# jyjblrd/Low-Cost-Mocap

Measured on AMD Instinct MI355X. Metric: triangulated 3D markers/sec at 8 cams x 16 markers, higher is better.
Workload: dtype f64

## Files before the change

### low-cost-mocap_amd/csrc/frame_bb.hip

```cpp
#include "mocap_device.hpp"
#include "kernels.hpp"
#include <cstdlib>
#include "frame_common.hpp"

namespace mocap {

constexpr int kBBThreads = 256;
constexpr int kBBWaves = kBBThreads / 64;
constexpr int kBBRecs = kBBThreads + 64;

constexpr int bb_wg_per_cu(int RL) { return RL == 48 ? 5 : 4; }
constexpr int kBBLdsSlack = 1024;
struct BBLayout {
  size_t bxy, bxy_nx, cnt_nx, bt, rbound, seedkey, slot_key, claimw, recs, rpk, scr, scr_bytes, goff, gcnt, outslot, boff, bnb, seedgh, slot_g, cnt,
      misc, bpl, nh, hits, act, root_blob, root_cam, nact, bnl, bv, bcache, bpk, total;
  int ncache;
  __host__ __device__ static size_t al(size_t x, size_t a) { return (x + a - 1) / a * a; }
  __host__ __device__ BBLayout(int C, int M, int R, int CW, int wg_per_cu) {
    size_t o = 0;
    auto take = [&](size_t bytes, size_t a) {
      o = al(o, a);
      const size_t at = o;
      o += bytes;
      return at;
    };
    bxy = take(sizeof(float2) * (size_t)C * M, 16);
    bxy_nx = take(sizeof(float2) * (size_t)C * M, 16);
    cnt_nx = take(4 * (size_t)C, 4);
    bt = take(sizeof(double) * 10 * ((size_t)C * M + 1), 16);
    rbound = take(8 * (size_t)R, 8);
    claimw = take(8 * (size_t)C, 8);
    scr = seedkey = take(8 * (size_t)R, 8);
    slot_key = take(8 * (size_t)kBBWaves * R, 8);
    recs = take(8 * (size_t)kBBRecs, 8);
    rpk = take(8 * (size_t)kBBRecs * CW, 8);
    seedgh = take(4 * (size_t)R, 4);
    slot_g = take(4 * (size_t)kBBWaves * R, 4);
    scr_bytes = o - scr;
    goff = take(4 * (size_t)(R + 1), 4);
    gcnt = take(4 * (size_t)R, 4);
    outslot = take(4 * (size_t)R, 4);
    boff = take(4 * (size_t)(R + 1), 4);
    bnb = take(4 * (size_t)R, 4);
    cnt = take(4 * (size_t)C, 4);
    misc = take(4 * 16, 4);
    bpl = take(2 * (size_t)R, 2);
    nh = take((size_t)R * C, 1);
    hits = take((size_t)R * C * M, 1);
    act = take((size_t)R * C, 1);
    root_blob = take((size_t)R, 1);
    root_cam = take((size_t)R, 1);
    nact = take((size_t)R, 1);
    bnl = take((size_t)R, 1);
    bv = take((size_t)R, 1);
    bcache = take(0, 8);
    ncache = 0;
    const size_t per_entry = 8 + 8 * (size_t)CW;
    for (int per_cu = wg_per_cu; per_cu >= 1; per_cu--) {
      const size_t lim = ((size_t)160 * 1024 / per_cu - kBBLdsSlack) / 256 * 256;
      if (lim >= o + per_entry * 64) {
        const size_t n = (lim - o) / per_entry;
        ncache = (int)(n > 1024 ? 1024 : n);
        break;
      }
    }
    o += 8 * (size_t)ncache;
    bpk = o;
    o += 8 * (size_t)CW * ncache;
    total = al(o, 16);
  }
};

static int bb_fixed_slots(int C, int M, int R) {
  const char* e = getenv("MOCAP_BB_FIXED_LAYOUT");
  if (e && e[0] == '0') return 0;
  if (C == 8 && M == 16 && R <= 48) return 48;
  if (C == 8 && M == 16 && R <= 64) return 64;
  return 0;
}
static int frame_bb_root_slots(int C, int M, int R) {
  const int f = bb_fixed_slots(C, M, R);
  return f ? f : R;
}
size_t frame_bb_lds_bytes(int C, int M, int R) { return BBLayout(C, M, frame_bb_root_slots(C, M, R), C <= 8 ? 1 : 2, bb_wg_per_cu(bb_fixed_slots(C, M, R))).total; }
static size_t frame_bb_lds_bytes_min(int C, int M, int R) {
  const BBLayout L(C, M, frame_bb_root_slots(C, M, R), C <= 8 ? 1 : 2, bb_wg_per_cu(bb_fixed_slots(C, M, R)));
  return L.total - (8 + 8 * (size_t)(C <= 8 ? 1 : 2)) * (size_t)L.ncache;
}
bool frame_bb_fits(int C, int M, int R) {
  return C >= 2 && C <= 16 && M >= 1 && M <= 64 && R >= 1 && R <= 255 && frame_bb_lds_bytes_min(C, M, R) <= (size_t)128 * 1024;
}

template <int CW>
struct Packed {
  unsigned long long w[CW];
  __device__ __forceinline__ void clear() {
#pragma unroll
    for (int k = 0; k < CW; k++) w[k] = ~0ull;
  }
  __device__ __forceinline__ void set(int c, uint32_t idx) {
    if (CW == 1)
      w[0] ^= (unsigned long long)(idx ^ 0xFFu) << (8 * c);
    else
      w[c >> 3] ^= (unsigned long long)(idx ^ 0xFFu) << (8 * (c & 7));
  }
  __device__ __forceinline__ uint32_t get(int c) const {
    return CW == 1 ? (uint32_t)(w[0] >> (8 * c)) & 0xFFu : (uint32_t)(w[c >> 3] >> (8 * (c & 7))) & 0xFFu;
  }
};

template <int CT>
struct BBCamTables {
  const double* base;
  static constexpr int C = CT;
  __device__ __forceinline__ ctab_t pq(size_t off) const { return as_ctab(base + off); }
  __device__ __forceinline__ ctab_t rt(size_t off) const { return as_ctab(base + 12 * CT + off); }
  __device__ __forceinline__ ctab_t k4(size_t off) const { return as_ctab(base + 24 * CT + off); }
  __device__ __forceinline__ const double* f() const { return base + 28 * CT; }
};
template <>
struct BBCamTables<0> {
  const double* base;
  int C;
  __device__ __forceinline__ ctab_t pq(size_t off) const { return as_ctab(base + off); }
  __device__ __forceinline__ ctab_t rt(size_t off) const { return as_ctab(base + 12 * C + off); }
  __device__ __forceinline__ ctab_t k4(size_t off) const { return as_ctab(base + 24 * C + off); }
  __device__ __forceinline__ const double* f() const { return base + 28 * C; }
};

enum { kPrioEval = 0, kPrioSeed = 1, kPrioPhase = 2, kPrioSerial = 3 };
template <int P>
__device__ __forceinline__ void bb_prio() {
  __builtin_amdgcn_s_setprio(P);
}

template <bool F32R, int CW, int CT, int ML, int RL>
struct BBState {
  static constexpr int T = kBBThreads, W = kBBWaves;
  const FrameArgs& p;
  BBCamTables<CT> cv;
  const int C_, M, R, RS;
  int tid, lane, wave;
  __device__ __forceinline__ void fresh_tid() {
    int t = tid;
    asm volatile("" : "+v"(t));
    tid = t;
    lane = t & 63;
    wave = t >> 6;
  }
  __device__ __forceinline__ int cn() const { return CT > 0 ? CT : C_; }
  double* bt;
  float2 *bxy, *bxy_nx;
  int32_t* cnt_nx;
  unsigned long long *rbound, *seedkey, *slot_key, *claimw, *rpk;
  struct BRec { uint32_t gh, rs; };
  BRec* recs;
  uint32_t *goff, *gcnt, *boff, *bnb, *seedgh, *slot_g;
  int32_t *outslot, *cnt, *misc;
  uint16_t* bpl;
  uint8_t *nh, *hits, *act, *root_blob, *root_cam, *nact, *bnl, *bv;
  float2* bcache;
  unsigned long long* bpk;
  int ncache;
  unsigned char* scr;
  size_t scr_bytes;
  static constexpr unsigned long long kInfBits = 0x7ff0000000000000ull;

  __device__ BBState(const FrameArgs& p_, unsigned char* smem)
      : p(p_), C_(p_.cv.C), M(ML > 0 ? ML : p_.M), R(p_.K_max), RS(RL > 0 ? RL : p_.K_max), tid(threadIdx.x), lane(threadIdx.x & 63), wave(threadIdx.x >> 6) {
    const int C = cn();
    {
      const unsigned long long ta = (unsigned long long)(uintptr_t)p_.cv.Pq;
      uint32_t tlo = (uint32_t)__builtin_amdgcn_readfirstlane((int)(uint32_t)ta);
      uint32_t thi = (uint32_t)__builtin_amdgcn_readfirstlane((int)(uint32_t)(ta >> 32));
      asm volatile("" : "+s"(tlo), "+s"(thi));
      cv.base = (const double*)(uintptr_t)(((unsigned long long)thi << 32) | tlo);
      if constexpr (CT == 0) cv.C = C;
    }
    const BBLayout L(C, M, RS, CW, bb_wg_per_cu(RL));
    bt = (double*)(smem + L.bt);
    bxy = (float2*)(smem + L.bxy);
    bxy_nx = (float2*)(smem + L.bxy_nx);
    cnt_nx = (int32_t*)(smem + L.cnt_nx);
    rbound = (unsigned long long*)(smem + L.rbound);
    seedkey = (unsigned long long*)(smem + L.seedkey);
    slot_key = (unsigned long long*)(smem + L.slot_key);
    claimw = (unsigned long long*)(smem + L.claimw);
    recs = (BRec*)(smem + L.recs);
    rpk = (unsigned long long*)(smem + L.rpk);
    goff = (uint32_t*)(smem + L.goff);
    gcnt = (uint32_t*)(smem + L.gcnt);
    outslot = (int32_t*)(smem + L.outslot);
    boff = (uint32_t*)(smem + L.boff);
    bnb = (uint32_t*)(smem + L.bnb);
    seedgh = (uint32_t*)(smem + L.seedgh);
    slot_g = (uint32_t*)(smem + L.slot_g);
    cnt = (int32_t*)(smem + L.cnt);
    misc = (int32_t*)(smem + L.misc);
    bpl = (uint16_t*)(smem + L.bpl);
    nh = (uint8_t*)(smem + L.nh);
    hits = (uint8_t*)(smem + L.hits);
    act = (uint8_t*)(smem + L.act);
    root_blob = (uint8_t*)(smem + L.root_blob);
    root_cam = (uint8_t*)(smem + L.root_cam);
    nact = (uint8_t*)(smem + L.nact);
    bnl = (uint8_t*)(smem + L.bnl);
    bv = (uint8_t*)(smem + L.bv);
    scr = smem + L.scr;
    scr_bytes = L.scr_bytes;
    bcache = (float2*)(smem + L.bcache);
    bpk = (unsigned long long*)(smem + L.bpk);
    ncache = L.ncache;
  }

  struct Line { double a, b, c, den, rden; };
  __device__ __forceinline__ Line epiline(int r, int i) const { return epiline_of(root_cam[r], root_blob[r], i); }
  __device__ __forceinline__ Line epiline_of(int rc, int rb, int i) const {
    const int C = cn();
    const double* Fm = cv.f() + 9 * ((size_t)rc * C + i);
    const float2 rp = bxy[(size_t)rc * M + rb];
    const double x = (double)rp.x, y = (double)rp.y;
    double a = Fm[0] * x + Fm[1] * y + Fm[2];
    double b = Fm[3] * x + Fm[4] * y + Fm[5];
    double c = Fm[6] * x + Fm[7] * y + Fm[8];
    double nu = a * a + b * b;
    nu = nu != 0.0 ? 1.0 / sqrt(nu) : 1.0;
    a *= nu;
    b *= nu;
    c *= nu;
    if (F32R) {
      a = (double)(float)a;
      b = (double)(float)b;
      c = (double)(float)c;
    }
    Line L;
    L.a = a;
    L.b = b;
    L.c = c;
    L.den = sqrt(a * a + b * b);
    L.rden = recip_refined(L.den);
    return L;
  }

  template <bool CHAIN>
  __device__ __forceinline__ unsigned long long match_pairs(const Line& mine, int pair_r, int pair_i, int n_pairs, int gs_shift,
                                                            int cam = 0, int Mi_chain = 0) {
    const int C = cn();
    const int GS = 1 << gs_shift, PPS = 64 >> gs_shift;
    const int k = lane & (GS - 1), q = lane >> gs_shift;
    const int gl0 = lane & ~(GS - 1);
    const unsigned long long gall = gs_shift == 6 ? ~0ull : ((1ull << GS) - 1ull);
    unsigned long long claims = 0ull;
    for (int s0 = 0; s0 < n_pairs; s0 += PPS) {
      const int src = s0 + q;
      const bool has = src < n_pairs;
      const int sl = has ? src : 0;
      const double la = __shfl(mine.a, sl), lb = __shfl(mine.b, sl), lc = __shfl(mine.c, sl);
      const double lden = __shfl(mine.den, sl), lrden = __shfl(mine.rden, sl);
      const int r = __shfl(pair_r, sl);
      const int i = CHAIN ? cam : __shfl(pair_i, sl);
      const int Mi = has ? (CHAIN ? Mi_chain : cnt[i]) : 0;
      const bool valid = k < Mi;
      float2 pt = make_float2(0.f, 0.f);
      double d = 0.0;
      bool hit = false;
      if (valid) {
        pt = bxy[(size_t)i * M + k];
        const double num = fabs(la * (double)pt.x + lb * (double)pt.y + lc);
        d = div_by(num, lden, lrden);
        hit = d < p.gate_px;
      }
      const unsigned long long wm = __ballot(hit);
      const unsigned long long gm = (wm >> gl0) & gall;
      int rank = 0;
      const unsigned int dlo = (unsigned int)__double_as_longlong(d), dhi = (unsigned int)(__double_as_longlong(d) >> 32);
      for (unsigned long long mm = wm; mm;) {
        const int j = __ffsll((long long)mm) - 1;
        mm &= mm - 1;
        const double dj = __longlong_as_double(((long long)__builtin_amdgcn_readlane((int)dhi, j) << 32) |
                                               (unsigned int)__builtin_amdgcn_readlane((int)dlo, j));
        const bool mine_grp = (j & ~(GS - 1)) == gl0 && j != lane;
        rank += (hit && mine_grp && (dj < d || (dj == d && j < lane))) ? 1 : 0;
      }
      if (hit) hits[((size_t)r * C + i) * M + rank] = (uint8_t)k;
      const unsigned long long g0 = (__ballot(hit && rank == 0) >> gl0) & gall;
      bool same = false;
      if (valid && g0) {
        const float2 p0 = bxy[(size_t)i * M + (__ffsll((long long)g0) - 1)];
        same = pt.x == p0.x && pt.y == p0.y;
      }
      const unsigned long long cw = __ballot(same);
      if (CHAIN) {
        for (int sh = 0; sh < 64; sh += GS) claims |= (cw >> sh) & gall;
      }
      if (has && k == 0) {
        nh[(size_t)r * C + i] = (uint8_t)__popcll(gm);
        if (!CHAIN) {
          const unsigned long long cm = (cw >> gl0) & gall;
          if (cm) atomicOr(&claimw[i], cm);
        }
      }
    }
    return claims;
  }

  __device__ __forceinline__ void prefetch_lds(int64_t frame) const {
    const int C = cn();
    const float* src = p.blobs + (size_t)frame * C * M * 2;
    const int n_dw = C * M * 2;
    for (int base = wave * 64; base < n_dw; base += T)
      if (base + lane < n_dw)
        __builtin_amdgcn_global_load_lds((const __attribute__((address_space(1))) void*)(src + base + lane),
                                         (__attribute__((address_space(3))) void*)((float*)bxy_nx + base), 4, 0, 0);
    if (wave == 0 && lane < C)
      __builtin_amdgcn_global_load_lds((const __attribute__((address_space(1))) void*)(p.counts + (size_t)frame * C + lane),
                                       (__attribute__((address_space(3))) void*)cnt_nx, 4, 0, 0);
  }
  __device__ __forceinline__ void stage(int64_t frame) {
    fresh_tid();
    const int C = cn();
    float2* t = bxy;
    bxy = bxy_nx;
    bxy_nx = t;
    if (tid < C) {
      const int n = cnt_nx[tid];
      cnt[tid] = n < 0 ? 0 : (n > M ? M : n);
      claimw[tid] = 0ull;
    }
    if (tid == 0) {
      misc[MI_STATUS] = 0;
      misc[MI_OMAX] = 0;
    }
  }

  __device__ void match() {
    fresh_tid();
    const int C = cn();
    __syncthreads();
    int gs_shift = 0;
    while ((1 << gs_shift) < M) gs_shift++;
    const int n0 = cnt[0] < R ? cnt[0] : R;
    {
      for (int r = tid; r < n0; r += T) {
        root_cam[r] = 0;
        root_blob[r] = (uint8_t)r;
      }
      if (tid == 0 && cnt[0] > R) misc[MI_STATUS] |= MOCAP_ST_ROOT_OVERFLOW_;
    }
    __syncthreads();
    auto U_of = [&](int j) {
      const int n = cnt[j];
      return ~claimw[j] & (n >= 64 ? ~0ull : ((1ull << n) - 1ull));
    };
    int n_prov = 0, n_ppairs = 0;
    bool pre = false;
    uint8_t* nh_s = nullptr;
    uint8_t* hits_s = nullptr;
    unsigned long long* pclaim = (unsigned long long*)scr;
    {
      int Mmax = 0;
      for (int c = 1; c < C; c++) Mmax = cnt[c] > Mmax ? cnt[c] : Mmax;
#pragma nounroll
      for (int stage_ = 0; stage_ < 2; stage_++) {
        const int stage = __builtin_amdgcn_readfirstlane(stage_);
        int NP = n0 * (C - 1);
        if (stage == 1) {
          block_sync_lds();
          for (int j = 1; j < C; j++) {
            const int np = __popcll(U_of(j));
            n_prov += np;
            n_ppairs += np * (C - 1 - j);
          }
          pre = n_prov <= 64 && (size_t)n_prov * C * (8 + 1 + (size_t)M) <= scr_bytes;
          if (!pre) break;
          nh_s = (uint8_t*)(pclaim + (size_t)n_prov * C);
          hits_s = nh_s + (size_t)n_prov * C;
          NP = n_ppairs;
        }
        for (int base = wave * 64; base < NP; base += W * 64) {
          const int pi = base + lane;
          const bool have = pi < NP;
          int r = 0, i = 1, Mi = 0;
          Line L = {0, 0, 0, 1, 1};
          if (have) {
            if (stage == 0) {
              r = pi / (C - 1);
              i = 1 + (pi - r * (C - 1));
              L = epiline(r, i);
            } else {
              int j = 1, acc = 0, pb = 0, span = C - 2;
              unsigned long long U = 0ull;
              for (; j <= C - 2; j++) {
                span = C - 1 - j;
                U = U_of(j);
                const int nj = __popcll(U) * span;
                if (pi < acc + nj) break;
                acc += nj;
                pb += __popcll(U);
              }
              uint32_t ord, off;
              divmod_tiny((uint32_t)(pi - acc), (uint32_t)span, ord, off);
              for (uint32_t t = 0; t < ord; t++) U &= U - 1;
              const int k = __ffsll((long long)U) - 1;
              i = j + 1 + (int)off;
              r = pb + (int)ord;
              L = epiline_of(j, k, i);
            }
            Mi = cnt[i];
          }
          const float2* pts = bxy + (size_t)i * M;
          auto dist = [&](int k) {
            const float2 pt = pts[k];
            return div_by(fabs(L.a * (double)pt.x + L.b * (double)pt.y + L.c), L.den, L.rden);
          };
          unsigned long long hm = 0ull;
#pragma unroll 4
          for (int k = 0; k < Mmax; k++)
            if (k < Mi && dist(k) < p.gate_px) hm |= 1ull << k;
          uint8_t* nhp = stage == 0 ? nh : nh_s;
          uint8_t* hl = (stage == 0 ? hits : hits_s) + ((size_t)r * C + i) * M;
          if (have) nhp[(size_t)r * C + i] = (uint8_t)__popcll(hm);
          unsigned long long rem = hm, claim = 0ull;
          int pos = 0;
          float2 p0 = make_float2(0.f, 0.f);
          while (__ballot(rem != 0ull)) {
            if (rem) {
              double bd = __builtin_huge_val();
              int bk = 0;
              for (unsigned long long t = rem; t; t &= t - 1) {
                const int k = __ffsll((long long)t) - 1;
                const double d = dist(k);
                if (d < bd) {
                  bd = d;
                  bk = k;
                }
              }
              hl[pos] = (uint8_t)bk;
              if (pos == 0) {
                p0 = pts[bk];
                for (unsigned long long t = hm; t; t &= t - 1) {
                  const int k = __ffsll((long long)t) - 1;
                  const float2 q = pts[k];
                  if (q.x == p0.x && q.y == p0.y) claim |= 1ull << k;
                }
              }
              rem &= ~(1ull << bk);
              pos++;
            }
          }
          if (stage == 0) {
            if (claim) atomicOr(&claimw[i], claim);
          } else if (have) {
            pclaim[(size_t)r * C + i] = claim;
          }
        }
      }
    }
    const int NL = M * ((C - 1) * (C - 2) / 2);
    const bool spec = F32R && (size_t)NL * 20 + 8 <= scr_bytes;
    double* sp_den = (double*)scr;
    float* sp_abc = (float*)(sp_den + NL);
    auto sp_base = [&](int j) { return M * ((j - 1) * (C - 1) - (j - 1) * j / 2); };
    if (spec && !pre) {
      int tot = 0;
      for (int j = 1; j <= C - 2; j++) {
        const int n = cnt[j];
        const unsigned long long U = ~claimw[j] & (n >= 64 ? ~0ull : ((1ull << n) - 1ull));
        tot += __popcll(U) * (C - 1 - j);
      }
      for (int l = tid; l < tot; l += T) {
        int j = 1, acc = 0, span = C - 2;
        unsigned long long U = 0ull;
        for (; j <= C - 2; j++) {
          const int n = cnt[j];
          U = ~claimw[j] & (n >= 64 ? ~0ull : ((1ull << n) - 1ull));
          span = C - 1 - j;
          const int nj = __popcll(U) * span;
          if (l < acc + nj) break;
          acc += nj;
        }
        uint32_t ord, off;
        divmod_tiny((uint32_t)(l - acc), (uint32_t)span, ord, off);
        for (uint32_t t = 0; t < ord; t++) U &= U - 1;
        const int k = __ffsll((long long)U) - 1, i = j + 1 + (int)off;
        const int ll = sp_base(j) + k * span + (int)off;
        const Line L = epiline_of(j, k, i);
        sp_den[ll] = L.den;
        sp_abc[3 * ll + 0] = (float)L.a;
        sp_abc[3 * ll + 1] = (float)L.b;
        sp_abc[3 * ll + 2] = (float)L.c;
      }
    }
    __syncthreads();
    fresh_tid();
    if (wave == 0) bb_prio<kPrioSerial>();
    if (wave == 0 && pre) {
      int jp = 0, kp = 0;
      if (lane < n_prov) {
        int acc = 0;
        unsigned long long U = 0ull;
        for (jp = 1; jp < C; jp++) {
          U = U_of(jp);
          const int np = __popcll(U);
          if (lane < acc + np) break;
          acc += np;
        }
        for (int t = 0; t < lane - acc; t++) U &= U - 1;
        kp = __ffsll((long long)U) - 1;
      }
      bool real = false;
      for (int i = 1; i < C; i++) {
        wave_lds_sync();
        if (lane < n_prov && jp == i) {
          real = !((claimw[i] >> kp) & 1ull);
          if (real)
            for (int c = i + 1; c < C; c++) {
              const unsigned long long m = pclaim[(size_t)lane * C + c];
              if (m) atomicOr(&claimw[c], m);
            }
        }
      }
      const unsigned long long rm = __ballot(real);
      const int rank = __popcll(rm & ((1ull << lane) - 1ull));
      int n_roots = n0 + __popcll(rm);
      if (real && n0 + rank < R) {
        root_cam[n0 + rank] = (uint8_t)jp;
        root_blob[n0 + rank] = (uint8_t)kp;
        bnl[rank] = (uint8_t)lane;
      }
      if (lane == 0) {
        if (n_roots > R) {
          misc[MI_STATUS] |= MOCAP_ST_ROOT_OVERFLOW_;
          n_roots = R;
        }
        misc[MI_NROOTS] = n_roots;
      }
    } else if (wave == 0) {
      const int cntL = lane < C ? cnt[lane] : 0;
      const unsigned long long clmL = lane < C ? claimw[lane] : 0ull;
      int nr_cam = 0, nr_blob = 0;
      int n_roots = n0;
      bool over = false;
      for (int i = 1; i < C; i++) {
        const int Mi = __builtin_amdgcn_readlane(cntL, i);
        unsigned long long claimed = ((unsigned long long)(unsigned int)__builtin_amdgcn_readlane((int)(clmL >> 32), i) << 32) |
                                     (unsigned int)__builtin_amdgcn_readlane((int)clmL, i);
        const int n_new = n_roots - n0;
        for (int base = 0; base < n_new; base += 64) {
          const int l = base + lane;
          const bool have = l < n_new;
          int j = nr_cam, k = nr_blob;
          if (base) {
            wave_lds_sync();
            j = have ? root_cam[n0 + l] : 0;
            k = have ? root_blob[n0 + l] : 0;
          }
          Line L = {0, 0, 0, 1, 1};
          if (have) {
            if (spec) {
              const int ll = sp_base(j) + k * (C - 1 - j) + (i - j - 1);
              L.a = (double)sp_abc[3 * ll + 0];
              L.b = (double)sp_abc[3 * ll + 1];
              L.c = (double)sp_abc[3 * ll + 2];
              L.den = sp_den[ll];
              L.rden = recip_refined(L.den);
            } else {
              L = epiline_of(j, k, i);
            }
          }
          claimed |= match_pairs<true>(L, n0 + l, i, (n_new - base < 64) ? n_new - base : 64, gs_shift, i, Mi);
        }
        const bool flag = lane < Mi && !((claimed >> lane) & 1ull);
        const unsigned long long mask = __ballot(flag);
        const int pos = __popcll(mask & ((1ull << lane) - 1ull));
        if (flag) {
          const int rr = n_roots + pos;
          if (rr < R) {
            root_cam[rr] = (uint8_t)i;
            root_blob[rr] = (uint8_t)lane;
          }
        }
        int slot = n_new;
        for (unsigned long long mm = mask; mm; slot++) {
          const int jb = __ffsll((long long)mm) - 1;
          mm &= mm - 1;
          if (lane == slot) {
            nr_cam = i;
            nr_blob = jb;
          }
        }
        n_roots += __popcll(mask);
        if (n_roots > R) {
          over = true;
          n_roots = R;
        }
      }
      if (lane == 0) {
        if (over) misc[MI_STATUS] |= MOCAP_ST_ROOT_OVERFLOW_;
        misc[MI_NROOTS] = n_roots;
      }
    } else {
      float om = 0.0f;
      for (int i = tid - 64; i < C * M; i += T - 64) {
        const int c = i / M, k = i - c * M;
        if (k < cnt[c]) {
          const float2 v = bxy[i];
          om = fmaxf(om, fmaxf(fabsf(v.x), fabsf(v.y)));
          double Bc[10];
          dlt_contribution(Bc, cv.pq(12 * c), (double)v.x, (double)v.y);
#pragma unroll
          for (int e = 0; e < 10; e++) bt[(size_t)i * 10 + e] = Bc[e];
        }
      }
      if (om > 0.0f) atomicMax(&misc[MI_OMAX], __float_as_int(om));
      if (tid == 64) {
        const int it = q_add(&p.q.counters[QC_NEXT_FRAME], 1);
        misc[MI_NEXT] = it < frame_count(p) ? it : -1;
      }
    }
    bb_prio<kPrioPhase>();
    __syncthreads();
    if (pre) {
      const int n_new = misc[MI_NROOTS] - n0;
      for (int idx = tid; idx < n_new * C; idx += T) {
        const int q = idx / C, c = idx - q * C;
        const int r = n0 + q, ps = bnl[q];
        if (c > (int)root_cam[r]) {
          const int n = nh_s[(size_t)ps * C + c];
          nh[(size_t)r * C + c] = (uint8_t)n;
          const uint8_t* src = hits_s + ((size_t)ps * C + c) * M;
          uint8_t* dst = hits + ((size_t)r * C + c) * M;
          for (int t = 0; t < n; t++) dst[t] = src[t];
        }
      }
      __syncthreads();
    }

    fresh_tid();
    const int nroots = misc[MI_NROOTS];
    for (int r = tid; r < nroots; r += T) {
      const int rc = root_cam[r];
      unsigned long long total = 1;
      int views = 1, na = 0;
      bool over = false;
      for (int c = rc + 1; c < C; c++) {
        const unsigned n = nh[(size_t)r * C + c];
        if (n > 1) act[(size_t)r * C + na++] = (uint8_t)c;
        if (n) {
          views++;
          total *= n;
          if (total > (unsigned long long)p.G_cap) {
            over = true;
            total = 1;
          }
        }
      }
      if (over) atomicOr(&misc[MI_STATUS], MOCAP_ST_CAND_OVERFLOW_);
      nact[r] = (uint8_t)na;
      bv[r] = (uint8_t)views;
      rbound[r] = kInfBits;
      const uint32_t g = (views > 1 && !over) ? (uint32_t)total : 0u;
      gcnt[r] = g;
      {
        const uint8_t* a = act + (size_t)r * C;
        uint32_t pl = 1, nb = 1;
        int nl = 0;
        while (nl < na && pl < (uint32_t)p.bb_pl) pl *= nh[(size_t)r * C + a[nl++]];
        for (int k = nl; k < na; k++) nb *= nh[(size_t)r * C + a[k]];
        bpl[r] = (uint16_t)pl;
        bnl[r] = (uint8_t)nl;
        bnb[r] = g ? nb : 0u;
        seedkey[r] = 0ull;
        seedgh[r] = 0xFFFFFFFFu;
      }
    }
    for (int s = tid; s < W * RS; s += T) {
      slot_key[s] = ~0ull;
      slot_g[s] = 0xFFFFFFFFu;
    }
    if (tid == 0) misc[MI_BBCTR] = misc[MI_BBCTR2] = 0;
    __syncthreads();
    if (wave == 0) bb_prio<kPrioSerial>();
    if (wave == 0) {
      uint32_t carry = 0, bcarry = 0;
      int slots = 0;
      for (int base = 0; base < nroots; base += 64) {
        const int r = base + lane;
        const uint32_t g = r < nroots ? gcnt[r] : 0u;
        const uint32_t nb = r < nroots ? bnb[r] : 0u;
        const uint32_t incl = wave_inclusive_scan(g, lane);
        const uint32_t bincl = wave_inclusive_scan(nb, lane);
        const unsigned long long nz = __ballot(g != 0u);
        if (r < nroots) {
          goff[r] = carry + incl - g;
          boff[r] = bcarry + bincl - nb;
          outslot[r] = g ? slots + __popcll(nz & ((1ull << lane) - 1ull)) : -1;
        }
        carry += (uint32_t)__builtin_amdgcn_readlane((int)incl, 63);
        bcarry += (uint32_t)__builtin_amdgcn_readlane((int)bincl, 63);
        slots += __popcll(nz);
      }
      if (lane == 0) {
        goff[nroots] = carry;
        boff[nroots] = bcarry;
        misc[MI_NOUT] = slots;
        misc[MI_G] = misc[MI_STATUS] ? 0 : (int32_t)carry;
      }
    }
    bb_prio<kPrioPhase>();
    __syncthreads();
  }

  template <bool WITH_B>
  __device__ __forceinline__ int group_matrix(int r, uint32_t rem, int skip, double (&B)[10], Packed<CW>& pk) const {
    const int C = cn();
    const int rc = root_cam[r];
    const uint8_t* nhr = nh + (size_t)r * C;
    const uint8_t* hr = hits + (size_t)r * C * M;
    pk.clear();
    int v = 0, ka = 0;
    if (WITH_B) {
#pragma unroll
      for (int e = 0; e < 10; e++) B[e] = 0.0;
    }
    for (int c = 0; c < C; c++) {
      uint32_t k = 0xFFu;
      if (c == rc) {
        k = root_blob[r];
      } else if (c > rc) {
        const uint32_t n = nhr[c];
        if (n == 1) {
          k = hr[(size_t)c * M];
        } else if (n > 1) {
          if (ka >= skip) {
            uint32_t qd, dgt;
            if (rem < 8192u) divmod_tiny(rem, n, qd, dgt); else
            divmod_small(rem, n, qd, dgt);
            rem = qd;
            k = hr[(size_t)c * M + dgt];
          }
          ka++;
        }
      }
      if (k != 0xFFu) {
        if (WITH_B) {
          const double* t = bt + ((size_t)c * M + k) * 10;
#pragma unroll
          for (int e = 0; e < 10; e++) B[e] = B[e] + t[e];
        }
        v++;
        pk.set(c, k);
      }
    }
    return v;
  }

  __device__ __forceinline__ int fetch_candidate(uint32_t lo, uint32_t i, int& r, uint32_t& gl, Packed<CW>& pk, double (&B)[10]) const {
    const int C = cn();
    const BRec rec = recs[lo];
    r = (int)(rec.rs & 0xFFu);
#pragma unroll
    for (int k = 0; k < CW; k++) pk.w[k] = rpk[(size_t)lo * CW + k];
    if (rec.rs >> 31) {
      gl = rec.gh;
    } else {
      uint32_t rem = i - (rec.rs >> 8);
      gl = rec.gh * (uint32_t)bpl[r] + rem;
      const uint8_t* a = act + (size_t)r * C;
      const int nl = bnl[r];
      for (int k = 0; k < nl; k++) {
        const int c = a[k];
        uint32_t qd, dgt;
        divmod_tiny(rem, nh[(size_t)r * C + c], qd, dgt);
        rem = qd;
        pk.set(c, hits[((size_t)r * C + c) * M + dgt]);
      }
    }
#pragma unroll
    for (int ee = 0; ee < 10; ee++) B[ee] = 0.0;
#pragma unroll CT > 0 ? CT : 1
    for (int c = 0; c < C; c++) {
      const uint32_t k = pk.get(c);
      const double* t = bt + (size_t)(k != 0xFFu ? (uint32_t)c * (uint32_t)M + k : (uint32_t)C * (uint32_t)M) * 10;
#pragma unroll
      for (int ee = 0; ee < 10; ee++) B[ee] = B[ee] + t[ee];
    }
    return bv[r];
  }

  __device__ void search(bool bound_tests) {
    fresh_tid();
    const int C = cn();
    (void)C;
    const int nroots = misc[MI_NROOTS];
    int32_t* ctr = &misc[MI_BBCTR];
    int32_t* ctr_other = &misc[MI_BBCTR2];
    const double inf = __builtin_huge_val();
    EigCut ec;
    {
      const double om = (double)__int_as_float(misc[MI_OMAX]);
      ec.p3max2 = p.p3max2;
      ec.o2slack = (1100.0 * 0x1p-46) * (om * om);
    }
    const double c0[3] = {p.bb_c0[0], p.bb_c0[1], p.bb_c0[2]};
    const uint32_t nblocks = boff[nroots];
    auto root_of_block = [&](uint32_t b_first_of_wave, uint32_t b) {
      return coop_last_le([&](int r) { return boff[r]; }, nroots, b_first_of_wave, b, lane);
    };
    auto push_block = [&](int r, uint32_t gh, const Packed<CW>& pk) {
      const uint32_t old = (uint32_t)atomicAdd(ctr, (int32_t)(((uint32_t)bpl[r] << 10) | 1u));
      const uint32_t slot = old & 0x3FFu;
      BRec rec;
      rec.gh = gh;
      rec.rs = (uint32_t)r | ((old >> 10) << 8);
      recs[slot] = rec;
#pragma unroll
      for (int k = 0; k < CW; k++) rpk[(size_t)slot * CW + k] = pk.w[k];
    };
    auto rec_start = [&](int k) { return (recs[k].rs & 0x7FFFFFFFu) >> 8; };
    auto dropped = [&](int r, double s1, double tr) {
      const int vf = bv[r];
      const double bound = __longlong_as_double((long long)rbound[r]);
      const double limit = bound * (double)(2 * vf) * (1.0 + 0x1p-40);
      const double limit_adj = fma(1.002, limit, (double)(2 * vf) * ec.o2slack);
      return s1 * fma(2e-12, tr, p.p3max2c * limit_adj) < 1.0;
    };
    if (bound_tests) {
      bb_prio<kPrioSeed>();
      int my_r = -1;
      uint32_t my_gh = 0;
      unsigned long long my_key = 0ull;
      Packed<CW> my_pk;
      my_pk.clear();
      for (uint32_t s0 = 0; s0 < nblocks; s0 += T) {
        const uint32_t b = s0 + (uint32_t)tid;
        if (s0 + (uint32_t)(wave * 64) >= nblocks) continue;
        const int r = root_of_block(s0 + (uint32_t)(wave * 64), b < nblocks ? b : nblocks - 1);
        if (b < nblocks) {
          const uint32_t gh = b - boff[r];
          double B[10], tr = 0.0;
          Packed<CW> pk;
          const int v = group_matrix<true>(r, gh, bnl[r], B, pk);
          double s1d = __builtin_huge_val();
          float s1 = 0.0f;
          if (v >= 2) {
            s1d = eigcut_s1_shifted(B, c0, tr);
            s1 = (float)fmin(s1d, 3e38);
          }
          if (b < (uint32_t)ncache) {
            bcache[b] = make_float2(__double2float_ru(s1d), __double2float_ru(tr));
#pragma unroll
            for (int k = 0; k < CW; k++) bpk[(size_t)b * CW + k] = pk.w[k];
          }
          my_key = ((unsigned long long)__float_as_uint(s1) << 32) | (unsigned long long)(0xFFFFFFFFu - gh);
          my_r = r;
          my_gh = gh;
          my_pk = pk;
          atomicMax(&seedkey[r], my_key);
        }
      }
      __syncthreads();
      if (nblocks <= (uint32_t)T) {
        if (my_r >= 0 && seedkey[my_r] == my_key) {
          seedgh[my_r] = my_gh;
          push_block(my_r, my_gh, my_pk);
        }
      } else
      for (int r = tid; r < nroots; r += T) {
        if (bnb[r]) {
          const uint32_t gh = 0xFFFFFFFFu - (uint32_t)seedkey[r];
          seedgh[r] = gh;
          seedkey[r] = 0ull;
          double B[10];
          Packed<CW> pk;
          group_matrix<false>(r, gh, bnl[r], B, pk);
          push_block(r, gh, pk);
        }
      }
      bb_prio<kPrioEval>();
      __syncthreads();
    }
    uint32_t b0 = 0;
    fresh_tid();
    while (true) {
      const uint32_t cv_ = (uint32_t)*ctr;
      const uint32_t ns = cv_ & 0x3FFu, ne = cv_ >> 10;
      const bool blocks_left = b0 < nblocks;
      const bool full = ns > (uint32_t)(kBBRecs - T);
      if (ns && (full || !blocks_left || ne >= (uint32_t)p.bb_flush)) {
        for (uint32_t i0 = 0; i0 < ne; i0 += T) {
          const uint32_t i = i0 + (uint32_t)tid;
          const bool have = i < ne;
          double e = inf, X[3] = {0, 0, 0};
          int r = 0;
          uint32_t gl = 0;
          uint32_t lo = 0;
          if (i0 + (uint32_t)(wave * 64) < ne)
            lo = (uint32_t)coop_last_le(rec_start, (int)ns, i0 + (uint32_t)(wave * 64), have ? i : ne - 1, lane);
          if (have) {
            Packed<CW> pk;
            double B[10];
            const int v = fetch_candidate(lo, i, r, gl, pk, B);
            auto obs_p = [&](int c, double& x, double& y) -> bool {
              const uint32_t k = pk.get(c);
              if (k == 0xFFu) return false;
              const float2 w = bxy[(size_t)c * M + k];
              x = (double)w.x;
              y = (double)w.y;
              return true;
            };
            const double bound = __longlong_as_double((long long)rbound[r]);
            solve_and_score<true, true, F32R, false>(cv, B, v, obs_p, X, e, bound * (double)(2 * v) * (1.0 + 0x1p-40), ec);
#ifdef MOCAP_DEBUG_EIGCHECK
            if (!(e < inf)) {
              double B2[10], X2[3], e2;
#pragma unroll
              for (int ee = 0; ee < 10; ee++) B2[ee] = 0.0;
              for (int c = 0; c < C; c++) {
                const uint32_t k = pk.get(c);
                if (k != 0xFFu) {
                  const double* t = bt + ((size_t)c * M + k) * 10;
#pragma unroll
                  for (int ee = 0; ee < 10; ee++) B2[ee] = B2[ee] + t[ee];
                }
              }
              solve_and_score<true, true, F32R>(cv, B2, v, obs_p, X2, e2);
              atomicAdd(&p.status[p.n_frames], 1);
              if (e2 <= bound) printf("EIGCHECK candidate: root %d g %u bound %.17g true %.17g\n", r, gl, bound, e2);
            }
#endif
          }
          const bool fin = e < inf;
          const unsigned long long key = fin ? (unsigned long long)__double_as_longlong(e) : kInfBits;
          const uint32_t gword = (gl << 1) | ((e != e) ? 1u : 0u);
          const int ss = wave * RS + r;
          if (fin) atomicMin(&rbound[r], key);
          const bool want = have && (key < slot_key[ss] || (key == slot_key[ss] && gword < slot_g[ss]));
          if (__ballot(want)) {
            unsigned long long old = 0;
            if (want) old = atomicMin(&slot_key[ss], key);
            wave_lds_sync();
            const bool holder = want && slot_key[ss] == key;
            if (holder && old > key) slot_g[ss] = 0xFFFFFFFFu;
            wave_lds_sync();
            if (holder) atomicMin(&slot_g[ss], gword);
            wave_lds_sync();
          }
        }
        __syncthreads();
        if (tid == 0) *ctr = 0;
        {
          int32_t* t = ctr;
          ctr = ctr_other;
          ctr_other = t;
        }
        continue;
      }
      if (!blocks_left) break;
      const uint32_t b = b0 + (uint32_t)tid;
      const uint32_t bw = b0 + (uint32_t)(wave * 64);
      b0 += T;
      int r = 0;
      if (bw < nblocks) r = root_of_block(bw, b < nblocks ? b : nblocks - 1);
      bool do_push = false;
      uint32_t gh = 0;
      Packed<CW> pk;
      pk.clear();
      if (b < nblocks) {
        gh = b - boff[r];
        if (gh != seedgh[r]) {
          double B[10], tr;
          bool survive = true;
          if (bound_tests && b < (uint32_t)ncache) {
            const float2 sc = bcache[b];
            survive = !dropped(r, (double)sc.x, (double)sc.y);
#pragma unroll
            for (int k = 0; k < CW; k++) pk.w[k] = bpk[(size_t)b * CW + k];
          } else if (bound_tests) {
            const int v = group_matrix<true>(r, gh, bnl[r], B, pk);
            if (v >= 2) {
              const double s1 = eigcut_s1_shifted(B, c0, tr);
              survive = !dropped(r, s1, tr);
            }
          } else {
            group_matrix<false>(r, gh, bnl[r], B, pk);
          }
          do_push = survive;
#ifdef MOCAP_DEBUG_EIGCHECK
          if (!survive) {
            const double bound = __longlong_as_double((long long)rbound[r]);
            const uint32_t pl = bpl[r];
            for (uint32_t l = 0; l < pl; l++) {
              double B2[10], X2[3], e2 = inf;
              Packed<CW> pk2;
              const int v2 = group_matrix<true>(r, gh * pl + l, 0, B2, pk2);
              auto obs2 = [&](int c, double& x, double& y) -> bool {
                const uint32_t k = pk2.get(c);
                if (k == 0xFFu) return false;
                const float2 w = bxy[(size_t)c * M + k];
                x = (double)w.x;
                y = (double)w.y;
                return true;
              };
              solve_and_score<true, true, F32R>(cv, B2, v2, obs2, X2, e2);
              atomicAdd(&p.status[p.n_frames + 1], 1);
              if (e2 <= bound) printf("EIGCHECK block: root %d block %u candidate %u bound %.17g true %.17g\n", r, gh, l, bound, e2);
            }
          }
#endif
        }
      }
      __syncthreads();
      if (do_push) push_block(r, gh, pk);
      __syncthreads();
    }
    __syncthreads();
  }

  __device__ bool root_winner(int r, double& eb, uint32_t& gb) const {
    if (!gcnt[r]) return false;
    unsigned long long kb = ~0ull;
    uint32_t gw = 0xFFFFFFFFu;
    for (int w = 0; w < W; w++) {
      const int s = w * RS + r;
      const unsigned long long k = slot_key[s];
      const uint32_t g = slot_g[s];
      if (k < kb || (k == kb && g < gw)) {
        kb = k;
        gw = g;
      }
    }
    if (kb == ~0ull) return false;
    gb = gw >> 1;
    eb = kb != kInfBits ? __longlong_as_double((long long)kb)
                        : ((gw & 1u) ? __longlong_as_double(0x7ff8000000000000ll) : __builtin_huge_val());
    return true;
  }

  __device__ void write_point(int64_t frame, int r, double e, uint32_t gl) const {
    const int C = cn();
    const size_t o = (size_t)frame * R + outslot[r];
    p.err[o] = e;
    double B[10];
#pragma unroll
    for (int ee = 0; ee < 10; ee++) B[ee] = 0.0;
    uint32_t rem = gl;
    const int rc = root_cam[r];
    int16_t* co = p.corr + o * C;
    for (int c = 0; c < C; c++) {
      int16_t s = -1;
      if (c == rc) {
        s = (int16_t)root_blob[r];
      } else if (c > rc) {
        const uint32_t n = nh[(size_t)r * C + c];
        if (n) {
          uint32_t qd = rem, dgt = 0;
          if (n > 1) {
            if (rem < 8192u) divmod_tiny(rem, n, qd, dgt); else
            divmod_small(rem, n, qd, dgt);
          }
          s = (int16_t)hits[((size_t)r * C + c) * M + dgt];
          rem = qd;
        }
      }
      co[c] = s;
      if (s >= 0) {
        const double* t = bt + ((size_t)c * M + (uint32_t)s) * 10;
#pragma unroll
        for (int ee = 0; ee < 10; ee++) B[ee] = B[ee] + t[ee];
      }
    }
    double X[3];
    solve_point(B, X);
    store_point(p, o, X);
  }
};

template <bool F32R, int CW, int CT, int ML, int RL>
__global__ __launch_bounds__(kBBThreads, bb_wg_per_cu(RL)) void frame_bb_kernel(FrameArgs p) {
  extern __shared__ __attribute__((aligned(16))) unsigned char smem[];
  BBState<F32R, CW, CT, ML, RL> st(p, smem);
  const int tid = threadIdx.x;
  const FrameQueues& q = p.q;
  if (tid == 0) {
    const int it = q_add(&q.counters[QC_NEXT_FRAME], 1);
    st.misc[MI_ITEM] = it < frame_count(p) ? it : -1;
  }
  if (tid < 10) st.bt[(size_t)st.cn() * st.M * 10 + tid] = 0.0;
  __syncthreads();
  int item = st.misc[MI_ITEM];
  if (item >= 0) st.prefetch_lds(item);
  wait_own_stores();
  __syncthreads();
  while (item >= 0) {
    const int64_t frame = item;
    bb_prio<kPrioPhase>();
    st.stage(frame);
    st.match();
    bb_prio<kPrioEval>();
    const int next = st.misc[MI_NEXT];
    if (next >= 0) st.prefetch_lds(next);
    if (tid == 0) {
      const int status = st.misc[MI_STATUS];
      p.n_out[frame] = status ? 0 : st.misc[MI_NOUT];
      p.status[frame] = status;
      if (p.n_cand) p.n_cand[frame] = st.misc[MI_G];
    }
    const uint32_t G = (uint32_t)st.misc[MI_G];
    if (G) {
      st.search(G >= (uint32_t)p.bb_min_g);
      bb_prio<kPrioPhase>();
      const int nroots = st.misc[MI_NROOTS];
      st.fresh_tid();
      for (int r = st.tid; r < nroots; r += kBBThreads) {
        if (st.outslot[r] < 0) continue;
        double e;
        uint32_t gl;
        if (st.root_winner(r, e, gl)) st.write_point(frame, r, e, gl);
      }
    }
    wait_own_stores();
    bb_prio<kPrioEval>();
    __syncthreads();
    item = next;
  }
  if (tid == 0 && q_add(&q.counters[QC_EXITED], 1) == (int)gridDim.x - 1)
    for (int c = 0; c < QC_COUNT; c++) q_store(&q.counters[c], 0);
}

int frame_bb_wg_per_cu_cap(int C, int M, int R) { return bb_wg_per_cu(bb_fixed_slots(C, M, R)); }
size_t frame_bb_ws_bytes(int) { return 0; }

hipError_t launch_frame_bb(const FrameArgs& a, int grid, hipStream_t stream) {
  const size_t lds = frame_bb_lds_bytes(a.cv.C, a.M, a.K_max);
  if (!a.cv.uniformK || a.cv.RT != a.cv.Pq + 12 * a.cv.C || a.cv.K4 != a.cv.Pq + 24 * a.cv.C || a.cv.F != a.cv.Pq + 28 * a.cv.C)
    return hipErrorInvalidValue;
  void (*k)(FrameArgs);
  const bool f32 = a.cv.f32_rounding != 0;
  const int fixed = bb_fixed_slots(a.cv.C, a.M, a.K_max);
  if (fixed == 48)
    k = f32 ? frame_bb_kernel<true, 1, 8, 16, 48> : frame_bb_kernel<false, 1, 8, 16, 48>;
  else if (fixed == 64)
    k = f32 ? frame_bb_kernel<true, 1, 8, 16, 64> : frame_bb_kernel<false, 1, 8, 16, 64>;
  else if (fixed)
    return hipErrorInvalidValue;
  else if (a.cv.C == 8)
    k = f32 ? frame_bb_kernel<true, 1, 8, 0, 0> : frame_bb_kernel<false, 1, 8, 0, 0>;
  else if (a.cv.C <= 8)
    k = f32 ? frame_bb_kernel<true, 1, 0, 0, 0> : frame_bb_kernel<false, 1, 0, 0, 0>;
  else
    k = f32 ? frame_bb_kernel<true, 2, 0, 0, 0> : frame_bb_kernel<false, 2, 0, 0, 0>;
  if (lds > 48 * 1024) {
    hipError_t e = hipFuncSetAttribute((const void*)k, hipFuncAttributeMaxDynamicSharedMemorySize, (int)lds);
    if (e != hipSuccess) return e;
  }
  hipLaunchKernelGGL(k, dim3(grid), dim3(kBBThreads), lds, stream, a);
  return hipGetLastError();
}

}
```

Baseline: 561.8 million.

## Compact LDS layout for 8x16 case: nibble-packed hits and single shared slot array

For the 48-root-slot 8-camera 16-marker configuration, hit indices are packed as 4-bit nibbles in one 64-bit word per root and camera, and the per-wave best-candidate slot arrays collapse into a single shared array guarded by a workgroup spinlock. The search scratch region is moved to the end of the layout so it can use all remaining LDS. The aim is to shrink LDS per workgroup so more cache entries fit, or occupancy holds at five workgroups per CU. The cost is extra bit manipulation on hit lookups, atomicOr writes, and serialization through the lock when waves update the winning slot.

```diff
diff --git a/low-cost-mocap_amd/csrc/frame_bb.hip b/low-cost-mocap_amd/csrc/frame_bb.hip
--- a/low-cost-mocap_amd/csrc/frame_bb.hip
+++ b/low-cost-mocap_amd/csrc/frame_bb.hip
@@ -10,13 +10,15 @@
 constexpr int kBBRecs = kBBThreads + 64;
 
 constexpr int bb_wg_per_cu(int RL) { return RL == 48 ? 5 : 4; }
+constexpr bool bb_compact(int RL) { return RL == 48; }
 constexpr int kBBLdsSlack = 1024;
+constexpr int kMiSlotLock = MI_HEAVY_N;
 struct BBLayout {
   size_t bxy, bxy_nx, cnt_nx, bt, rbound, seedkey, slot_key, claimw, recs, rpk, scr, scr_bytes, goff, gcnt, outslot, boff, bnb, seedgh, slot_g, cnt,
       misc, bpl, nh, hits, act, root_blob, root_cam, nact, bnl, bv, bcache, bpk, total;
   int ncache;
   __host__ __device__ static size_t al(size_t x, size_t a) { return (x + a - 1) / a * a; }
-  __host__ __device__ BBLayout(int C, int M, int R, int CW, int wg_per_cu) {
+  __host__ __device__ BBLayout(int C, int M, int R, int CW, int wg_per_cu, bool compact) {
     size_t o = 0;
     auto take = [&](size_t bytes, size_t a) {
       o = al(o, a);
@@ -24,19 +26,23 @@
       o += bytes;
       return at;
     };
+    const int SW = compact ? 1 : kBBWaves;
     bxy = take(sizeof(float2) * (size_t)C * M, 16);
     bxy_nx = take(sizeof(float2) * (size_t)C * M, 16);
     cnt_nx = take(4 * (size_t)C, 4);
     bt = take(sizeof(double) * 10 * ((size_t)C * M + 1), 16);
     rbound = take(8 * (size_t)R, 8);
     claimw = take(8 * (size_t)C, 8);
-    scr = seedkey = take(8 * (size_t)R, 8);
-    slot_key = take(8 * (size_t)kBBWaves * R, 8);
-    recs = take(8 * (size_t)kBBRecs, 8);
-    rpk = take(8 * (size_t)kBBRecs * CW, 8);
-    seedgh = take(4 * (size_t)R, 4);
-    slot_g = take(4 * (size_t)kBBWaves * R, 4);
-    scr_bytes = o - scr;
+    auto take_search = [&]() {
+      scr = seedkey = take(8 * (size_t)R, 8);
+      slot_key = take(8 * (size_t)SW * R, 8);
+      recs = take(8 * (size_t)kBBRecs, 8);
+      rpk = take(8 * (size_t)kBBRecs * CW, 8);
+      seedgh = take(4 * (size_t)R, 4);
+      slot_g = take(4 * (size_t)SW * R, 4);
+      scr_bytes = o - scr;
+    };
+    if (!compact) take_search();
     goff = take(4 * (size_t)(R + 1), 4);
     gcnt = take(4 * (size_t)R, 4);
     outslot = take(4 * (size_t)R, 4);
@@ -46,13 +52,14 @@
     misc = take(4 * 16, 4);
     bpl = take(2 * (size_t)R, 2);
     nh = take((size_t)R * C, 1);
-    hits = take((size_t)R * C * M, 1);
+    hits = compact ? take((size_t)R * C * 8, 8) : take((size_t)R * C * M, 1);
     act = take((size_t)R * C, 1);
     root_blob = take((size_t)R, 1);
     root_cam = take((size_t)R, 1);
     nact = take((size_t)R, 1);
     bnl = take((size_t)R, 1);
     bv = take((size_t)R, 1);
+    if (compact) take_search();
     bcache = take(0, 8);
     ncache = 0;
     const size_t per_entry = 8 + 8 * (size_t)CW;
@@ -68,6 +75,7 @@
     bpk = o;
     o += 8 * (size_t)CW * ncache;
     total = al(o, 16);
+    if (compact) scr_bytes = total - scr;
   }
 };
 
@@ -82,9 +90,13 @@
   const int f = bb_fixed_slots(C, M, R);
   return f ? f : R;
 }
-size_t frame_bb_lds_bytes(int C, int M, int R) { return BBLayout(C, M, frame_bb_root_slots(C, M, R), C <= 8 ? 1 : 2, bb_wg_per_cu(bb_fixed_slots(C, M, R))).total; }
+static BBLayout frame_bb_layout(int C, int M, int R) {
+  const int f = bb_fixed_slots(C, M, R);
+  return BBLayout(C, M, frame_bb_root_slots(C, M, R), C <= 8 ? 1 : 2, bb_wg_per_cu(f), bb_compact(f));
+}
+size_t frame_bb_lds_bytes(int C, int M, int R) { return frame_bb_layout(C, M, R).total; }
 static size_t frame_bb_lds_bytes_min(int C, int M, int R) {
-  const BBLayout L(C, M, frame_bb_root_slots(C, M, R), C <= 8 ? 1 : 2, bb_wg_per_cu(bb_fixed_slots(C, M, R)));
+  const BBLayout L = frame_bb_layout(C, M, R);
   return L.total - (8 + 8 * (size_t)(C <= 8 ? 1 : 2)) * (size_t)L.ncache;
 }
 bool frame_bb_fits(int C, int M, int R) {
@@ -137,6 +149,9 @@
 template <bool F32R, int CW, int CT, int ML, int RL>
 struct BBState {
   static constexpr int T = kBBThreads, W = kBBWaves;
+  static constexpr bool NIB = bb_compact(RL);
+  static_assert(!NIB || (ML == 16 && CT > 0), "the compact layout is the 8 x 16 one");
+  static constexpr int SW = NIB ? 1 : W;
   const FrameArgs& p;
   BBCamTables<CT> cv;
   const int C_, M, R, RS;
@@ -165,6 +180,10 @@
   unsigned char* scr;
   size_t scr_bytes;
   static constexpr unsigned long long kInfBits = 0x7ff0000000000000ull;
+  __device__ __forceinline__ unsigned long long* hits64() const { return (unsigned long long*)hits; }
+  __device__ __forceinline__ uint32_t nib_hit(int r, int c, uint32_t t) const {
+    return (((const uint32_t*)hits)[((size_t)r * cn() + c) * 2 + (t >> 3)] >> (4 * (t & 7))) & 0xFu;
+  }
 
   __device__ BBState(const FrameArgs& p_, unsigned char* smem)
       : p(p_), C_(p_.cv.C), M(ML > 0 ? ML : p_.M), R(p_.K_max), RS(RL > 0 ? RL : p_.K_max), tid(threadIdx.x), lane(threadIdx.x & 63), wave(threadIdx.x >> 6) {
@@ -177,7 +196,7 @@
       cv.base = (const double*)(uintptr_t)(((unsigned long long)thi << 32) | tlo);
       if constexpr (CT == 0) cv.C = C;
     }
-    const BBLayout L(C, M, RS, CW, bb_wg_per_cu(RL));
+    const BBLayout L(C, M, RS, CW, bb_wg_per_cu(RL), NIB);
     bt = (double*)(smem + L.bt);
     bxy = (float2*)(smem + L.bxy);
     bxy_nx = (float2*)(smem + L.bxy_nx);
@@ -282,7 +301,14 @@
         const bool mine_grp = (j & ~(GS - 1)) == gl0 && j != lane;
         rank += (hit && mine_grp && (dj < d || (dj == d && j < lane))) ? 1 : 0;
       }
-      if (hit) hits[((size_t)r * C + i) * M + rank] = (uint8_t)k;
+      if constexpr (NIB) {
+        uint32_t* hw = (uint32_t*)hits64() + ((size_t)r * C + i) * 2;
+        if (has && k == 0) hits64()[(size_t)r * C + i] = 0ull;
+        wave_lds_sync();
+        if (hit) atomicOr(&hw[rank >> 3], (uint32_t)k << (4 * (rank & 7)));
+      } else {
+        if (hit) hits[((size_t)r * C + i) * M + rank] = (uint8_t)k;
+      }
       const unsigned long long g0 = (__ballot(hit && rank == 0) >> gl0) & gall;
       bool same = false;
       if (valid && g0) {
@@ -371,10 +397,15 @@
             n_prov += np;
             n_ppairs += np * (C - 1 - j);
           }
-          pre = n_prov <= 64 && (size_t)n_prov * C * (8 + 1 + (size_t)M) <= scr_bytes;
+          pre = n_prov <= 64 && (size_t)n_prov * C * (8 + 1 + (size_t)(NIB ? 8 : M)) <= scr_bytes;
           if (!pre) break;
-          nh_s = (uint8_t*)(pclaim + (size_t)n_prov * C);
-          hits_s = nh_s + (size_t)n_prov * C;
+          if constexpr (NIB) {
+            hits_s = (uint8_t*)(pclaim + (size_t)n_prov * C);
+            nh_s = hits_s + (size_t)n_prov * C * 8;
+          } else {
+            nh_s = (uint8_t*)(pclaim + (size_t)n_prov * C);
+            hits_s = nh_s + (size_t)n_prov * C;
+          }
           NP = n_ppairs;
         }
         for (int base = wave * 64; base < NP; base += W * 64) {
@@ -418,7 +449,8 @@
           for (int k = 0; k < Mmax; k++)
             if (k < Mi && dist(k) < p.gate_px) hm |= 1ull << k;
           uint8_t* nhp = stage == 0 ? nh : nh_s;
-          uint8_t* hl = (stage == 0 ? hits : hits_s) + ((size_t)r * C + i) * M;
+          uint8_t* hl = (stage == 0 ? hits : hits_s) + ((size_t)r * C + i) * (NIB ? 8 : M);
+          unsigned long long row = 0ull;
           if (have) nhp[(size_t)r * C + i] = (uint8_t)__popcll(hm);
           unsigned long long rem = hm, claim = 0ull;
           int pos = 0;
@@ -435,7 +467,10 @@
                   bk = k;
                 }
               }
-              hl[pos] = (uint8_t)bk;
+              if constexpr (NIB)
+                row |= (unsigned long long)bk << (4 * pos);
+              else
+                hl[pos] = (uint8_t)bk;
               if (pos == 0) {
                 p0 = pts[bk];
                 for (unsigned long long t = hm; t; t &= t - 1) {
@@ -448,6 +483,7 @@
               pos++;
             }
           }
+          if (NIB && have) *(unsigned long long*)hl = row;
           if (stage == 0) {
             if (claim) atomicOr(&claimw[i], claim);
           } else if (have) {
@@ -628,9 +664,13 @@
         if (c > (int)root_cam[r]) {
           const int n = nh_s[(size_t)ps * C + c];
           nh[(size_t)r * C + c] = (uint8_t)n;
-          const uint8_t* src = hits_s + ((size_t)ps * C + c) * M;
-          uint8_t* dst = hits + ((size_t)r * C + c) * M;
-          for (int t = 0; t < n; t++) dst[t] = src[t];
+          if constexpr (NIB) {
+            hits64()[(size_t)r * C + c] = ((const unsigned long long*)hits_s)[(size_t)ps * C + c];
+          } else {
+            const uint8_t* src = hits_s + ((size_t)ps * C + c) * M;
+            uint8_t* dst = hits + ((size_t)r * C + c) * M;
+            for (int t = 0; t < n; t++) dst[t] = src[t];
+          }
         }
       }
       __syncthreads();
@@ -674,7 +714,7 @@
         seedgh[r] = 0xFFFFFFFFu;
       }
     }
-    for (int s = tid; s < W * RS; s += T) {
+    for (int s = tid; s < SW * RS; s += T) {
       slot_key[s] = ~0ull;
       slot_g[s] = 0xFFFFFFFFu;
     }
@@ -730,14 +770,14 @@
       } else if (c > rc) {
         const uint32_t n = nhr[c];
         if (n == 1) {
-          k = hr[(size_t)c * M];
+          k = NIB ? nib_hit(r, c, 0) : hr[(size_t)c * M];
         } else if (n > 1) {
           if (ka >= skip) {
             uint32_t qd, dgt;
             if (rem < 8192u) divmod_tiny(rem, n, qd, dgt); else
             divmod_small(rem, n, qd, dgt);
             rem = qd;
-            k = hr[(size_t)c * M + dgt];
+            k = NIB ? nib_hit(r, c, dgt) : hr[(size_t)c * M + dgt];
           }
           ka++;
         }
@@ -773,7 +813,7 @@
         uint32_t qd, dgt;
         divmod_tiny(rem, nh[(size_t)r * C + c], qd, dgt);
         rem = qd;
-        pk.set(c, hits[((size_t)r * C + c) * M + dgt]);
+        pk.set(c, NIB ? nib_hit(r, c, dgt) : hits[((size_t)r * C + c) * M + dgt]);
       }
     }
 #pragma unroll
@@ -933,18 +973,27 @@
           const bool fin = e < inf;
           const unsigned long long key = fin ? (unsigned long long)__double_as_longlong(e) : kInfBits;
           const uint32_t gword = (gl << 1) | ((e != e) ? 1u : 0u);
-          const int ss = wave * RS + r;
+          const int ss = NIB ? r : wave * RS + r;
           if (fin) atomicMin(&rbound[r], key);
-          const bool want = have && (key < slot_key[ss] || (key == slot_key[ss] && gword < slot_g[ss]));
+          const bool want = have && (NIB ? key <= slot_key[ss] : (key < slot_key[ss] || (key == slot_key[ss] && gword < slot_g[ss])));
           if (__ballot(want)) {
+            if (NIB && lane == 0) {
+              while (atomicCAS(&misc[kMiSlotLock], 0, 1) != 0) __builtin_amdgcn_s_sleep(1);
+            }
+            if (NIB) __builtin_amdgcn_fence(__ATOMIC_ACQUIRE, "workgroup");
+            const bool want2 = NIB ? want && (key < slot_key[ss] || (key == slot_key[ss] && gword < slot_g[ss])) : want;
             unsigned long long old = 0;
-            if (want) old = atomicMin(&slot_key[ss], key);
+            if (want2) old = atomicMin(&slot_key[ss], key);
             wave_lds_sync();
-            const bool holder = want && slot_key[ss] == key;
+            const bool holder = want2 && slot_key[ss] == key;
             if (holder && old > key) slot_g[ss] = 0xFFFFFFFFu;
             wave_lds_sync();
             if (holder) atomicMin(&slot_g[ss], gword);
             wave_lds_sync();
+            if (NIB) {
+              __builtin_amdgcn_fence(__ATOMIC_RELEASE, "workgroup");
+              if (lane == 0) atomicExch(&misc[kMiSlotLock], 0);
+            }
           }
         }
         __syncthreads();
@@ -1021,7 +1070,7 @@
     if (!gcnt[r]) return false;
     unsigned long long kb = ~0ull;
     uint32_t gw = 0xFFFFFFFFu;
-    for (int w = 0; w < W; w++) {
+    for (int w = 0; w < SW; w++) {
       const int s = w * RS + r;
       const unsigned long long k = slot_key[s];
       const uint32_t g = slot_g[s];
@@ -1059,7 +1108,7 @@
             if (rem < 8192u) divmod_tiny(rem, n, qd, dgt); else
             divmod_small(rem, n, qd, dgt);
           }
-          s = (int16_t)hits[((size_t)r * C + c) * M + dgt];
+          s = (int16_t)(NIB ? nib_hit(r, c, dgt) : hits[((size_t)r * C + c) * M + dgt]);
           rem = qd;
         }
       }
@@ -1087,6 +1136,7 @@
     st.misc[MI_ITEM] = it < frame_count(p) ? it : -1;
   }
   if (tid < 10) st.bt[(size_t)st.cn() * st.M * 10 + tid] = 0.0;
+  if (tid == 0 && st.NIB) st.misc[kMiSlotLock] = 0;
   __syncthreads();
   int item = st.misc[MI_ITEM];
   if (item >= 0) st.prefetch_lds(item);
```

After: 567.1 million, median of 6. No clear change (+0.9%).
